# wustl-cig/FLAIR

Hardware: AMD Instinct MI355X
Metric: restored frames/sec at 256x256, 16-frame clip, 250-step DDIM (higher is better)
Workload: dtype bf16

## Files before the change

flair_amd/csrc/ew.hip:

```cpp
#include "common.h"

namespace {

template <typename E>
__global__ void nchw_to_nhwc_kernel(const float* src, int N, int C, long HW, E* dst, int ld, int coff) {
    const long total = (long)N * HW;
    for (long i = blockIdx.x * (long)blockDim.x + threadIdx.x; i < total; i += (long)gridDim.x * blockDim.x) {
        const long n = i / HW, p = i % HW;
        for (int c = 0; c < C; ++c) ET<E>::st(dst + i * ld + coff + c, src[(n * C + c) * HW + p]);
    }
}

template <typename E>
__global__ void nhwc_to_nchw_kernel(const E* src, int ld, int coff, int N, int C, long HW, float* dst) {
    const long total = (long)N * HW;
    for (long i = blockIdx.x * (long)blockDim.x + threadIdx.x; i < total; i += (long)gridDim.x * blockDim.x) {
        const long n = i / HW, p = i % HW;
        for (int c = 0; c < C; ++c) dst[(n * C + c) * HW + p] = ET<E>::ld(src + i * ld + coff + c);
    }
}

__global__ void timestep_embedding_kernel(const float* t, int N, int dim, float maxPeriod, int sinFirst,
                                          float* out) {
    const int half = dim / 2;
    const int i = blockIdx.x * blockDim.x + threadIdx.x;
    if (i >= N * half) return;
    const int n = i / half, k = i % half;
    const float freq = expf(-logf(maxPeriod) * (float)k / (float)half);
    const float arg = t[n] * freq;
    out[(long)n * dim + (sinFirst ? half : 0) + k] = cosf(arg);
    out[(long)n * dim + (sinFirst ? 0 : half) + k] = sinf(arg);
    if ((dim & 1) && k == 0) out[(long)n * dim + dim - 1] = 0.f;
}

template <int MMAX>
__global__ void linear_f32_kernel(const float* x, int M, int K, const float* w, const float* b, int N, int fpw,
                                  int actIn, int actOut, float* y, int yLd) {
    extern __shared__ float xs[];
    for (int i = threadIdx.x; i < M * K; i += blockDim.x) xs[i] = apply_act(x[i], actIn);
    __syncthreads();
    const int lane = threadIdx.x & 63;
    const int n0 = (blockIdx.x * (blockDim.x >> 6) + (threadIdx.x >> 6)) * fpw;
    for (int n = n0; n < n0 + fpw && n < N; ++n) {
        float acc[MMAX];
#pragma unroll
        for (int m = 0; m < MMAX; ++m) acc[m] = 0.f;
        const float* wr = w + (long)n * K;
        for (int k0 = lane; k0 < K; k0 += 64 * 8) {
            float wv[8];
#pragma unroll
            for (int j = 0; j < 8; ++j) wv[j] = k0 + 64 * j < K ? wr[k0 + 64 * j] : 0.f;
#pragma unroll
            for (int j = 0; j < 8; ++j) {
                const int k = k0 + 64 * j < K ? k0 + 64 * j : 0;
#pragma unroll
                for (int m = 0; m < MMAX; ++m)
                    if (m < M) acc[m] = fmaf(xs[m * K + k], wv[j], acc[m]);
            }
        }
#pragma unroll
        for (int m = 0; m < MMAX; ++m) {
            float v = acc[m];
#pragma unroll
            for (int off = 32; off > 0; off >>= 1) v += __shfl_xor(v, off);
            if (lane == 0 && m < M) y[(long)m * yLd + n] = apply_act(v + (b ? b[n] : 0.f), actOut);
        }
    }
}

__global__ void predict_xstart_kernel(const float* x, const float* modelOut, int N, int C, int Cm, long HW,
                                      float cRecip, float cRecipm1, int clip, float* x0) {
    const long total = (long)N * C * HW;
    for (long i = blockIdx.x * (long)blockDim.x + threadIdx.x; i < total; i += (long)gridDim.x * blockDim.x) {
        const long n = i / (C * HW), r = i % (C * HW);
        const float eps = modelOut[n * Cm * HW + r];
        float v = cRecip * x[i] - cRecipm1 * eps;
        if (clip) v = fminf(fmaxf(v, -1.f), 1.f);
        x0[i] = v;
    }
}

__global__ void sampler_update_kernel(const float* x, float* x0, const float* restored, const float* aux,
                                      const float* z, const float* prev, long frameElems, int T, int Tp,
                                      long total, float gamma, float wAux, float cRecip,
                                      float cRecipm1, float cPrev, float coNoise, float sq1mRho, float sqRho,
                                      int clip, int nonzero, float* xPrev) {
    for (long i = blockIdx.x * (long)blockDim.x + threadIdx.x; i < total; i += (long)gridDim.x * blockDim.x) {
        float v = x0[i];
        if (restored) {
            v = v - gamma * restored[i];
            if (clip) v = fminf(fmaxf(v, -1.f), 1.f);
        }
        if (aux) {
            float f = aux[i];
            if (clip) f = fminf(fmaxf(f, -1.f), 1.f);
            v = wAux * v + (1.f - wAux) * f;
        }
        if (prev) {
            const long n = i / frameElems, r = i % frameElems;
            const long b = n / T;
            const int t = (int)(n % T);
            if (t < Tp) v = prev[(b * Tp + t) * frameElems + r];
        }
        x0[i] = v;
        const float xi = x[i];
        const float eps = (cRecip * xi - v) / cRecipm1;
        float out = cPrev * v;
        if (nonzero) out += sq1mRho * coNoise * eps + sqRho * coNoise * z[i];
        xPrev[i] = out;
    }
}

__global__ void axpby_kernel(const float* x, const float* y, float a, float b, float lo, float hi, long n,
                             float* out) {
    for (long i = blockIdx.x * (long)blockDim.x + threadIdx.x; i < n; i += (long)gridDim.x * blockDim.x)
        out[i] = fminf(fmaxf(a * x[i] + (y ? b * y[i] : 0.f), lo), hi);
}

template <typename E>
__global__ void scale_pixels_kernel(E* x, int ld, int C, long P, const float* wmap) {
    constexpr int VEC = ET<E>::VEC;
    const int cv = C / VEC;
    const long total = P * cv;
    for (long i = blockIdx.x * (long)blockDim.x + threadIdx.x; i < total; i += (long)gridDim.x * blockDim.x) {
        const long p = i / cv;
        const int c0 = (int)(i % cv) * VEC;
        float v[VEC];
        Vec16<E>::load(x + p * ld + c0, v);
        const float s = wmap[p];
#pragma unroll
        for (int k = 0; k < VEC; ++k) v[k] *= s;
        Vec16<E>::store(x + p * ld + c0, v);
    }
}


__global__ void affine_channels_kernel(const float* x, int xLd, int C, long P, float a, float b, float lo,
                                       float hi, const float* sub, const float* mul, float* y, int yLd) {
    const long total = P * C;
    for (long i = blockIdx.x * (long)blockDim.x + threadIdx.x; i < total; i += (long)gridDim.x * blockDim.x) {
        const long p = i / C;
        const int c = (int)(i % C);
        float v = fminf(fmaxf(x[p * xLd + c] * a + b, lo), hi);
        y[p * yLd + c] = (v - (sub ? sub[c] : 0.f)) * (mul ? mul[c] : 1.f);
    }
}

template <typename E>
__global__ void add_frame_bias_kernel(E* x, int ld, int C, int F, long HW, const float* bias, int bLd) {
// ... 53 lines not shown
            Vec16<E>::load(x1 + p * ld1 + c0, b);
#pragma unroll
            for (int k = 0; k < VEC; ++k) a[k] += b[k];
        }
#pragma unroll
        for (int k = 0; k < VEC; ++k) a[k] = apply_act(a[k], act);
        Vec16<E>::store(y + p * yLd + c0, a);
    }
}

template <typename E>
__global__ void maxpool3s2_kernel(const E* x, int xLd, int F, int H, int W, int C, E* y, int yLd) {
    constexpr int VEC = ET<E>::VEC;
    const int cv = C / VEC, Ho = (H + 1) / 2, Wo = (W + 1) / 2;
    const long total = (long)F * Ho * Wo * cv;
    for (long i = blockIdx.x * (long)blockDim.x + threadIdx.x; i < total; i += (long)gridDim.x * blockDim.x) {
        const int c0 = (int)(i % cv) * VEC;
        long q = i / cv;
        const int wo = (int)(q % Wo);
        q /= Wo;
        const int ho = (int)(q % Ho), f = (int)(q / Ho);
        float m[VEC];
#pragma unroll
        for (int k = 0; k < VEC; ++k) m[k] = -INFINITY;
        for (int dh = -1; dh <= 1; ++dh) {
            const int h = 2 * ho + dh;
            if ((unsigned)h >= (unsigned)H) continue;
            for (int dw = -1; dw <= 1; ++dw) {
                const int w = 2 * wo + dw;
                if ((unsigned)w >= (unsigned)W) continue;
                float v[VEC];
                Vec16<E>::load(x + (((long)f * H + h) * W + w) * xLd + c0, v);
#pragma unroll
                for (int k = 0; k < VEC; ++k) m[k] = fmaxf(m[k], v[k]);
            }
        }
        Vec16<E>::store(y + (((long)f * Ho + ho) * Wo + wo) * yLd + c0, m);
    }
}

}

extern "C" int flair_nchw_f32_to_nhwc(const float* src, int N, int C, int H, int W, void* dst, int dtype,
                                      int dst_ld, int dst_coff, hipStream_t stream) {
    FLAIR_CHECK(src && dst && N > 0 && C > 0 && H > 0 && W > 0 && dst_coff >= 0 && dst_coff + C <= dst_ld,
                "flair_nchw_f32_to_nhwc: bad argument");
    const long HW = (long)H * W;
    return flair_by_dtype("flair_nchw_f32_to_nhwc", dtype, [&](auto e) -> int {
        using E = decltype(e);
        hipLaunchKernelGGL(nchw_to_nhwc_kernel<E>, dim3(grid_for(N * HW, 256, 2048)), dim3(256), 0, stream, src, N, C, HW,
                           (E*)dst, dst_ld, dst_coff);
        FLAIR_LAUNCH_CHECK();
        return FLAIR_OK;
    });
}

extern "C" int flair_nhwc_to_nchw_f32(const void* src, int dtype, int src_ld, int src_coff, int N, int C, int H,
                                      int W, float* dst, hipStream_t stream) {
    FLAIR_CHECK(src && dst && N > 0 && C > 0 && H > 0 && W > 0 && src_coff >= 0 && src_coff + C <= src_ld,
                "flair_nhwc_to_nchw_f32: bad argument");
    const long HW = (long)H * W;
    return flair_by_dtype("flair_nhwc_to_nchw_f32", dtype, [&](auto e) -> int {
        using E = decltype(e);
        hipLaunchKernelGGL(nhwc_to_nchw_kernel<E>, dim3(grid_for(N * HW, 256, 2048)), dim3(256), 0, stream,
                           (const E*)src, src_ld, src_coff, N, C, HW, dst);
        FLAIR_LAUNCH_CHECK();
        return FLAIR_OK;
    });
}

extern "C" int flair_timestep_embedding(const float* t, int N, int dim, float max_period, int sin_first,
                                        float* out, hipStream_t stream) {
    FLAIR_CHECK(t && out && N > 0 && dim >= 2, "flair_timestep_embedding: bad argument");
    const int n = N * (dim / 2);
    hipLaunchKernelGGL(timestep_embedding_kernel, dim3((n + 255) / 256), dim3(256), 0, stream, t, N, dim, max_period,
                       sin_first, out);
    FLAIR_LAUNCH_CHECK();
    return FLAIR_OK;
}

extern "C" int flair_linear_f32(const float* x, int M, int K, const float* w, const float* bias, int N, int act_in,
                                int act_out, float* y, int y_ld, hipStream_t stream) {
    FLAIR_CHECK(x && w && y && M > 0 && M <= 32 && K > 0 && N > 0 && y_ld >= N, "flair_linear_f32: bad argument (M<=32)");
    const size_t lds = (size_t)M * K * sizeof(float);
    FLAIR_CHECK(lds <= 64 * 1024, "flair_linear_f32: M*K too large for LDS staging");
    const int wavesPerBlock = 4;
    const int fpw = N >= 8192 ? 8 : 1;
    const int grid = (N + wavesPerBlock * fpw - 1) / (wavesPerBlock * fpw);
    if (M <= 8)
        hipLaunchKernelGGL(linear_f32_kernel<8>, dim3(grid), dim3(256), lds, stream, x, M, K, w, bias, N, fpw,
                           act_in, act_out, y, y_ld);
    else if (M <= 16)
        hipLaunchKernelGGL(linear_f32_kernel<16>, dim3(grid), dim3(256), lds, stream, x, M, K, w, bias, N, fpw,
                           act_in, act_out, y, y_ld);
    else
        hipLaunchKernelGGL(linear_f32_kernel<32>, dim3(grid), dim3(256), lds, stream, x, M, K, w, bias, N, fpw,
                           act_in, act_out, y, y_ld);
    FLAIR_LAUNCH_CHECK();
    return FLAIR_OK;
}

extern "C" int flair_predict_xstart(const float* x, const float* model_out, int N, int C, int Cm, int H, int W,
                                    float c_recip, float c_recipm1, int clip, float* x0, hipStream_t stream) {
    FLAIR_CHECK(x && model_out && x0 && N > 0 && C > 0 && Cm >= C, "flair_predict_xstart: bad argument");
    const long HW = (long)H * W;
    hipLaunchKernelGGL(predict_xstart_kernel, dim3(grid_for((long)N * C * HW, 256, 2048)), dim3(256), 0, stream, x, model_out, N,
                       C, Cm, HW, c_recip, c_recipm1, clip, x0);
    FLAIR_LAUNCH_CHECK();
    return FLAIR_OK;
}

extern "C" int flair_sampler_update(const flair_sampler_coefs* c, const float* x, float* x0, const float* restored,
                                    const float* aux, const float* z, const float* prev_recon, long n,
                                    float* x_prev, hipStream_t stream) {
    FLAIR_CHECK(c && x && x0 && x_prev && n > 0, "flair_sampler_update: null argument");
    FLAIR_CHECK(!c->nonzero || z, "flair_sampler_update: noise required when t != 0");
    FLAIR_CHECK(!prev_recon || (c->frame_elems > 0 && c->frames > 0 && c->prev_frames > 0 &&
                                c->prev_frames <= c->frames && n % (c->frame_elems * c->frames) == 0),
                "flair_sampler_update: prev_recon geometry");
    hipLaunchKernelGGL(sampler_update_kernel, dim3(grid_for(n, 256, 2048)), dim3(256), 0, stream, x, x0, restored, aux, z,
                       prev_recon, (long)c->frame_elems, c->frames, c->prev_frames, n,
                       c->gamma, c->w_aux, c->sqrt_recip_alphas_cumprod, c->sqrt_recipm1_alphas_cumprod,
                       c->sqrt_alphas_cumprod_prev, c->sqrt_one_minus_alphas_cumprod_prev, c->sqrt_one_minus_rho,
                       c->sqrt_rho, c->clip_denoised, c->nonzero, x_prev);
    FLAIR_LAUNCH_CHECK();
    return FLAIR_OK;
}

extern "C" int flair_axpby_f32(const float* x, const float* y, float a, float b, float lo, float hi, long n,
                               float* out, hipStream_t stream) {
    FLAIR_CHECK(x && out && n > 0, "flair_axpby_f32: bad argument");
    hipLaunchKernelGGL(axpby_kernel, dim3(grid_for(n, 256, 2048)), dim3(256), 0, stream, x, y, a, b, lo, hi, n, out);
    FLAIR_LAUNCH_CHECK();
    return FLAIR_OK;
}

extern "C" int flair_scale_pixels(void* x, int dtype, int ld, int C, long P, const float* wmap, hipStream_t stream) {
    FLAIR_CHECK(x && wmap && P > 0 && C > 0, "flair_scale_pixels: bad argument");
    return flair_by_dtype("flair_scale_pixels", dtype, [&](auto e) -> int {
        using E = decltype(e);
        constexpr int VEC = ET<E>::VEC;
        FLAIR_CHECK_VIEW("flair_scale_pixels", "x", x, ld, C, VEC);
        FLAIR_CHECK(C % VEC == 0, "flair_scale_pixels: C %% %d", VEC);
        hipLaunchKernelGGL(scale_pixels_kernel<E>, dim3(grid_for(P * (C / VEC), 256, 2048)), dim3(256), 0, stream, (E*)x, ld, C, P,
                           wmap);
        FLAIR_LAUNCH_CHECK();
        return FLAIR_OK;
    });
}

extern "C" int flair_affine_channels_f32(const float* x, int x_ld, int C, long P, float a, float b, float lo,
                                         float hi, const float* sub, const float* mul, float* y, int y_ld,
                                         hipStream_t stream) {
    FLAIR_CHECK(x && y && C > 0 && P > 0 && x_ld >= C && y_ld >= C, "flair_affine_channels_f32: bad argument");
    hipLaunchKernelGGL(affine_channels_kernel, dim3(grid_for(P * C, 256, 2048)), dim3(256), 0, stream, x, x_ld, C, P, a, b, lo,
                       hi, sub, mul, y, y_ld);
    FLAIR_LAUNCH_CHECK();
    return FLAIR_OK;
}

extern "C" int flair_add_frame_bias(void* x, int dtype, int ld, int C, int F, long HW, const float* bias,
                                    int bias_ld, hipStream_t stream) {
    FLAIR_CHECK(x && bias && C > 0 && F > 0 && HW > 0 && ld >= C && bias_ld >= C, "flair_add_frame_bias: bad argument");
    return flair_by_dtype("flair_add_frame_bias", dtype, [&](auto e) -> int {
        using E = decltype(e);
        hipLaunchKernelGGL(add_frame_bias_kernel<E>, dim3(grid_for(F * HW * C, 256, 2048)), dim3(256), 0, stream, (E*)x, ld, C, F,
                           HW, bias, bias_ld);
        FLAIR_LAUNCH_CHECK();
        return FLAIR_OK;
    });
}

extern "C" int flair_cast_channels(const float* src, int src_ld, int C, long P, void* dst, int dtype, int dst_ld,
                                   int dst_coff, hipStream_t stream) {
    FLAIR_CHECK(src && dst && C > 0 && P > 0 && src_ld >= C && dst_coff >= 0 && dst_coff + C <= dst_ld,
                "flair_cast_channels: bad argument");
    return flair_by_dtype("flair_cast_channels", dtype, [&](auto e) -> int {
        using E = decltype(e);
        hipLaunchKernelGGL(cast_channels_kernel<E>, dim3(grid_for(P * C, 256, 2048)), dim3(256), 0, stream, src, src_ld, C, P,
                           (E*)dst, dst_ld, dst_coff);
        FLAIR_LAUNCH_CHECK();
// ... 82 lines not shown
```

flair_amd/guided_diffusion/clip_model.py:

```python
import torch

from .packing import PackedModel


class ClipModel(PackedModel):

    _name = "flair_amd.ClipModel"

    def __init__(self, *args, **kwargs):
        super().__init__(*args, **kwargs)
        self._flow_cache = {}
        self._graphs = {}
        self.use_hip_graph = False
        self._flow_gen = 0
        self._trace = None

    def enable_hip_graph(self, flag=True):
        self.use_hip_graph = bool(flag)
        self._graphs = {}
        return self

    convert_to_fp16 = PackedModel.convert_to_bf16

    def invalidate_packed(self):
        super().invalidate_packed()
        self._graphs, self._flow_cache = {}, {}

    def reset_flow_cache(self):
        self._flow_cache = {}
        self._flow_gen += 1

    def _flows_cached(self, rnn_clip, spec):
        key = (rnn_clip.data_ptr(), rnn_clip._version, tuple(rnn_clip.shape), spec)
        hit = self._flow_cache.get(key)
        if hit is None:
            flows = self._compute_flows(rnn_clip, spec)
            flows["_prop"] = {}
            if len(self._flow_cache) >= 16:
                self._flow_cache.clear()
            hit = (flows, rnn_clip)
            self._flow_cache[key] = hit
        return hit[0]

    def _clip_flows(self, rnn_clip, x, enable_cross_frames):
        spec = self._flow_spec(x.shape[-2], x.shape[-1], enable_cross_frames)
        return self._flows_cached(rnn_clip, spec) if spec else {}

    def _run_clips(self, x, timesteps, low_res_input, rnn_input, num_frames, enable_cross_frames, vsrpp_weights):
        if not x.is_cuda:
            raise RuntimeError(f"{self._name} runs on the MI355X only (tensors must be on 'cuda'); "
                               "there is no CPU path")
        self._ensure_packed(x.device)
        T = int(num_frames)
        B = x.shape[0] // T
        if rnn_input is None:
            rnn_input = low_res_input
        graphed = self.use_hip_graph and self._trace is None
        outs = []
        for b in range(B):
            xb, tb = (v[b * T:(b + 1) * T].float().contiguous() for v in (x, timesteps))
            lr, rnn = (v[b].float().contiguous() for v in (low_res_input, rnn_input))
            vw = vsrpp_weights[b] if isinstance(vsrpp_weights, torch.Tensor) else vsrpp_weights
            if graphed:
                outs.append(self._forward_clip_graphed(xb, tb, lr, rnn, enable_cross_frames, vw, b))
            else:
                outs.append(self._forward_clip(xb, tb, lr, self._clip_flows(rnn, xb, enable_cross_frames),
                                               enable_cross_frames, vw))
        return outs[0] if B == 1 else torch.cat(outs, dim=0)

    def _forward_clip_graphed(self, x, t, low_res, rnn, enable_cross_frames, vsrpp_weights, clip):
        vw_t = vsrpp_weights if isinstance(vsrpp_weights, torch.Tensor) else None
        key = (tuple(x.shape), self.dtype, bool(enable_cross_frames),
               tuple(vw_t.shape) if vw_t is not None else vsrpp_weights, x.device, clip)
        src = (rnn.data_ptr(), rnn._version, low_res.data_ptr(), low_res._version, self._flow_gen,
               (vw_t.data_ptr(), vw_t._version) if vw_t is not None else None)
        ent = self._graphs.get(key)
        if ent is not None and ent["src"] != src:
            del self._graphs[key]
            ent = None
        if ent is None:
            st = dict(x=x.clone(), t=t.clone(), lr=low_res.clone(), rnn=rnn.clone(),
                      vw=vw_t.clone() if vw_t is not None else vsrpp_weights)
            flows = self._clip_flows(st["rnn"], x, enable_cross_frames)
            args = (st["x"], st["t"], st["lr"], flows, enable_cross_frames, st["vw"])
            cur = torch.cuda.current_stream()
            side = torch.cuda.Stream()
            side.wait_stream(cur)
            with torch.cuda.stream(side):
                self._forward_clip(*args)
            cur.wait_stream(side)
            torch.cuda.synchronize()
            graph = torch.cuda.CUDAGraph()
            with torch.cuda.graph(graph, capture_error_mode="thread_local"):
                out = self._forward_clip(*args)
            ent = dict(graph=graph, st=st, out=out, src=src, flows=flows)
            self._graphs[key] = ent
        ent["st"]["x"].copy_(x)
        ent["st"]["t"].copy_(t)
        ent["graph"].replay()
        return ent["out"]
```

flair_amd/guided_diffusion/sr3.py:

```python
import numpy as np
import torch
import torch.nn as nn

from .. import ops
from .clip_model import ClipModel
from .nn_new import linear, zero_module
from .packing import LinearStack, dev_f32, pack_w, packed_conv, pk_int, run_conv
from .unet_new import A, BasicVSRPP, Ctx, PlaceHolder, SPyNet, TemporalAttention, normalization

LazyReshaper2D = LazyReshaper3D = PlaceHolder


def aa_bilinear_table(n_in, n_out):
    scale = n_in / n_out
    support = scale if scale >= 1.0 else 1.0
    inv = 1.0 / scale if scale >= 1.0 else 1.0
    rows_i, rows_w = [], []
    for i in range(n_out):
        center = scale * (i + 0.5)
        lo = max(int(center - support + 0.5), 0)
        hi = min(int(center + support + 0.5), n_in)
        js = np.arange(lo, hi)
        w = np.clip(1.0 - np.abs((js - center + 0.5) * inv), 0.0, None).astype(np.float32)
        w = w / w.sum()
# ... 251 lines not shown
        self._shared_spynet = [shared]
        e = inner_channel
        self.noise_level_mlp = nn.Sequential(PositionalEncoding(inner_channel), nn.Linear(inner_channel, inner_channel * 4),
                                             Swish(), nn.Linear(inner_channel * 4, inner_channel))

        def blk(cin, cout, res):
            return ResnetBlocWithAttn(
                cin, cout, noise_level_emb_dim=e, norm_groups=norm_groups, dropout=dropout, conv_3d=cross_frame_module,
                temporal_attn=(res in attn_res and temporal_attn and cross_frame_module), num_frames=num_frames,
                head_dim=head_dim, vsrpp=(res in vsrpp_res and cross_frame_module),
                shared_spynet=shared if (res in vsrpp_res and cross_frame_module) else None)

        pre, res = inner_channel, image_size
        feats = [pre]
        downs = [LazyReshaper2D(nn.Conv2d(in_channel, inner_channel, kernel_size=3, padding=1))]
        n = len(channel_mults)
        for i in range(n):
            ch = inner_channel * channel_mults[i]
            for _ in range(res_blocks):
                downs.append(blk(pre, ch, res))
                feats.append(ch)
                pre = ch
            if i != n - 1:
                downs.append(LazyReshaper2D(Downsample(pre)))
                feats.append(pre)
                res //= 2
        self.downs = nn.ModuleList(downs)
        mk = dict(noise_level_emb_dim=e, norm_groups=norm_groups, dropout=dropout, conv_3d=cross_frame_module,
                  temporal_attn=temporal_attn and cross_frame_module, num_frames=num_frames, head_dim=head_dim)
        self.mid = nn.ModuleList([ResnetBlocWithAttn(pre, pre, **mk), ResnetBlocWithAttn(pre, pre, **mk)])
        ups, self._skip_split = [], {}
        for i in reversed(range(n)):
            ch = inner_channel * channel_mults[i]
            for _ in range(res_blocks + 1):
                skip = feats.pop()
                b = blk(pre + skip, ch, res)
                self._skip_split[id(b.res_block)] = [pre, skip]
                ups.append(b)
                pre = ch
            if i >= 1:
                ups.append(LazyReshaper2D(Upsample(pre)))
                res *= 2
        self.ups = nn.ModuleList(ups)
        self.final_conv = Block(pre, out_channel if out_channel is not None else in_channel, groups=norm_groups)

    def _pack_all(self, dt, device):
        stem = self.downs[0].wrapped_module
        stem._pk = packed_conv(stem, None, dt, device)
        plain, silu = LinearStack(), LinearStack()
        for m in self.modules():
            if isinstance(m, ResnetBlock):
                m.pack(dt, device, self._skip_split.get(id(m)), plain_off=plain.add(m.noise_func.noise_func[0]))
            elif isinstance(m, (ResBlock, TemporalWrapper2)):
                m.pack(dt, device, silu_off=silu.add(m.emb_layers[1]))
            elif isinstance(m, (TemporalAttention, BasicVSRPP, Downsample, Upsample)):
                m.pack(dt, device)
        if self._shared_spynet[0] is not None:
            self._shared_spynet[0].to(device)
            self._shared_spynet[0].pack(dt, device)
        mlp, fc = self.noise_level_mlp, self.final_conv.block
        self._pk = dict(
            plain=plain.cat(device), silu=silu.cat(device),
            mlp=[dev_f32(p, device) for p in (mlp[1].weight, mlp[1].bias, mlp[3].weight, mlp[3].bias)],
            fin_g=dev_f32(fc[0].wrapped_module.weight, device), fin_b=dev_f32(fc[0].wrapped_module.bias, device),
            fin=packed_conv(fc[3].wrapped_module, None, dt, device))
        self._flow_cache = {}

    def _flow_spec(self, H, W, enable_cross_frames):
        return tuple(self._flow_resolutions(H, W)) if enable_cross_frames else ()

    def _compute_flows(self, rnn_clip, resolutions):
        flows = {}
        for rh, r in resolutions:
            src = rnn_clip if tuple(rnn_clip.shape[-2:]) == (rh, r) else aa_resize(rnn_clip, (rh, r))
            raw = torch.zeros((src.shape[0], rh, r, 4), dtype=torch.float32, device=src.device)
            ops.nchw_to_clip(src.contiguous(), raw, 0)
            flows[r] = self._shared_spynet[0].pair_flows(raw)
        return flows

    def forward(self, x, timesteps, low_res_input=None, rnn_input=None, num_frames=None,
                enable_cross_frames=True, vsrpp_weights=None, **kwargs):
        return self._run_clips(x, timesteps, low_res_input, rnn_input, num_frames, enable_cross_frames, vsrpp_weights)

    def _forward_clip(self, x, level, low_res, flows, enable_cross_frames, vsrpp_weights):
        T, _, H, W = x.shape
        dev, dt = x.device, self.dtype
        ctx = Ctx(dt, dev, T)
        ctx.enable_cross_frames = enable_cross_frames
        ctx.vsrpp_weights = vsrpp_weights
        ctx.flows = flows
        pe = ops.timestep_embedding(level, self.inner_channel, sin_first=True)
        pk = self._pk
        e = ops.linear(pe, pk["mlp"][0], pk["mlp"][1], act_out=A.ACT_SILU)
        emb = ops.linear(e, pk["mlp"][2], pk["mlp"][3])
        ctx.plain_all = ops.linear(emb, pk["plain"][0], pk["plain"][1])
        ctx.silu_all = ops.linear(emb, pk["silu"][0], pk["silu"][1], act_in=A.ACT_SILU)
        cin = ops.pad_channels(self.in_channel, dt)
        h = torch.zeros((T, H, W, cin), dtype=dt, device=dev)
        ops.nchw_to_clip(low_res, h, 0)
        ops.nchw_to_clip(x, h, low_res.shape[1])
        feats = []
        for layer in self.downs:
            h = self._run_layer(ctx, layer, h)
            feats.append(h)
        for layer in self.mid:
            h = layer.run(ctx, h)
        for layer in self.ups:
            if isinstance(layer, ResnetBlocWithAttn):
                h = layer.run(ctx, h, feats.pop())
            else:
                h = self._run_layer(ctx, layer, h)
        fc = self.final_conv
        h = ops.group_norm(h, pk["fin_g"], pk["fin_b"], groups=fc.groups, eps=fc.block[0].wrapped_module.eps, act=A.ACT_SILU)
        y = run_conv(h, pk["fin"], fc.block[3].wrapped_module)
        return ops.clip_to_nchw(y, fc.block[3].wrapped_module.out_channels)

    def _flow_resolutions(self, H, W):
        hs, ws = ([r for r, _ in self._vsrpp_levels(n)] for n in (H, W))
        return sorted(set(zip(hs, ws)), key=lambda p: p[1])

    def _vsrpp_levels(self, size):
        out, res = [], size
        for layer in self.downs:
            if isinstance(layer, ResnetBlocWithAttn):
                if hasattr(layer, "vsrpp"):
                    out.append((res, layer.vsrpp.wrapped_module))
            elif isinstance(layer.wrapped_module, Downsample):
                res //= 2
        for layer in self.ups:
            if isinstance(layer, ResnetBlocWithAttn):
                if hasattr(layer, "vsrpp"):
                    out.append((res, layer.vsrpp.wrapped_module))
            elif isinstance(layer.wrapped_module, Upsample):
                res *= 2
        return out

    def _run_layer(self, ctx, layer, h):
        if isinstance(layer, ResnetBlocWithAttn):
            return layer.run(ctx, h)
        inner = layer.wrapped_module
        if isinstance(inner, nn.Conv2d):
            return run_conv(h, inner._pk, inner)
        if isinstance(inner, (Downsample, Upsample)):
            return inner.run(h)
        raise TypeError(f"flair_amd: no executor for {type(inner).__name__}")
```

flair_amd/guided_diffusion/unet_new.py:

```python
import math

import torch
import torch.nn as nn

from .. import ops
from .clip_model import ClipModel
from .nn_new import conv_nd, linear, normalization, zero_module
from .packing import LinearStack, dev_f32, pack_w, packed_conv, pk_int, run_conv

A = ops


class PlaceHolder(nn.Module):

    def __init__(self, module):
        super().__init__()
        self.wrapped_module = module


LazyReshaper2D = LazyReshaper3D = PlaceHolder


class TemporalWrapper(PlaceHolder):
    """unet_new.py:50-59 (skipped when ``enable_cross_frames`` is False)."""


class Ctx:

    def __init__(self, dtype, device, T):
        self.dtype, self.device, self.T = dtype, device, T
        self.emb = None
        self.film_all = None
        self.flows = {}
        self.vsrpp_weights = None
        self.enable_cross_frames = True


class ResBlock(nn.Module):

    def __init__(self, channels, emb_channels, dropout, out_channels=None, use_conv=False,
                 use_scale_shift_norm=False, dims=2, use_checkpoint=False, up=False, down=False):
        super().__init__()
        if not use_scale_shift_norm:
            raise NotImplementedError("flair_amd: only use_scale_shift_norm=True (the shipped "
                                      "FLAIR configuration) is implemented")
        if use_conv:
            raise NotImplementedError("flair_amd: 3x3 skip convolutions are not used by FLAIR")
        self.channels = channels
        self.out_channels = out_channels or channels
        self.dims, self.up, self.down = dims, up, down
        self.in_layers = nn.Sequential(
            PlaceHolder(normalization(channels)), nn.SiLU(),
            PlaceHolder(conv_nd(dims, channels, self.out_channels, 3, padding=1)))
        self.emb_layers = nn.Sequential(nn.SiLU(), linear(emb_channels, 2 * self.out_channels))
        self.out_layers = nn.Sequential(
            PlaceHolder(normalization(self.out_channels)), nn.SiLU(), nn.Dropout(p=dropout),
            zero_module(PlaceHolder(conv_nd(dims, self.out_channels, self.out_channels, 3, padding=1))))
        if self.out_channels == channels:
            self.skip_connection = nn.Identity()
        else:
            self.skip_connection = PlaceHolder(conv_nd(dims, channels, self.out_channels, 1))

    film_off = pk_int("film_off")

    def pack(self, dtype, device, split=None, film_off=0):
        c, co = self.channels, self.out_channels
        segs = [(s, s) for s in (split or [c])]
        self._pk = dict(
            film_off=film_off,
            w1=pack_w(self.in_layers[2].wrapped_module.weight, dtype, device, [(c, c)]),
            b1=dev_f32(self.in_layers[2].wrapped_module.bias, device),
            w2=pack_w(self.out_layers[3].wrapped_module.weight, dtype, device, [(co, co)]),
            b2=dev_f32(self.out_layers[3].wrapped_module.bias, device),
            g1=dev_f32(self.in_layers[0].wrapped_module.weight, device),
            be1=dev_f32(self.in_layers[0].wrapped_module.bias, device),
            g2=dev_f32(self.out_layers[0].wrapped_module.weight, device),
            be2=dev_f32(self.out_layers[0].wrapped_module.bias, device))
        if not isinstance(self.skip_connection, nn.Identity):
            self._pk["ws"] = pack_w(self.skip_connection.wrapped_module.weight, dtype, device, segs)
            self._pk["bs"] = dev_f32(self.skip_connection.wrapped_module.bias, device)

    def run(self, ctx, x, x1=None):
        pk = self._pk
        co = self.out_channels
        k = (1, 3, 3) if self.dims == 2 else (3, 3, 3)
        film = ctx.film_all[:, pk["film_off"]:pk["film_off"] + 2 * co]
        eps = self.in_layers[0].wrapped_module.eps
        if self.up or self.down:
            assert x1 is None
            h, x = ops.group_norm(x, pk["g1"], pk["be1"], eps=eps, act=A.ACT_SILU,
                                  resample=2 if self.up else 1, want_raw=True)
        else:
            h = ops.group_norm(x, pk["g1"], pk["be1"], x1=x1, eps=eps, act=A.ACT_SILU)
        h = ops.conv(h, pk["w1"], pk["b1"], co, k)
        h = ops.group_norm(h, pk["g2"], pk["be2"], eps=eps, act=A.ACT_SILU, film=film)
        if "ws" in pk:
            skip = ops.conv([x] if x1 is None else [x, x1], pk["ws"], pk["bs"], co, (1, 1, 1))
        else:
            assert x1 is None
            skip = x
        return ops.conv(h, pk["w2"], pk["b2"], co, k, res0=skip)


QKV_ATTN_WIDTHS = (32, 64, 128)


def qkv_head_width(channels, num_heads):
    d = channels // num_heads if num_heads > 0 and channels % num_heads == 0 else 0
    if d <= 0 or d % 8:
        raise NotImplementedError(f"flair_amd: attention head width {channels}/{num_heads} unsupported "
                                  f"({QKV_ATTN_WIDTHS} and multiples of 64 from 192 to 1024 at any size, other "
                                  "multiples of 8 while width + H*W <= 2048)")
    return d


def temporal_head_width(channels, num_heads):
    d = channels // num_heads if num_heads > 0 and channels % num_heads == 0 else 0
    if d < 8 or d > 256 or d % 8:
# ... 141 lines not shown
                    w1=pack_w(rb.conv1.weight, dtype, device, [(c, c)]), b1=dev_f32(rb.conv1.bias, device),
                    w2=pack_w(rb.conv2.weight, dtype, device, [(c, c)]), b2=dev_f32(rb.conv2.bias, device))




def run_trunk(pk, segs, c, *, extra_res=None, out=None, out_scale=1.0):
    k = (1, 3, 3)
    t1 = ops.conv(segs, pk["w0"], pk["b0"], c, k, act=A.ACT_LRELU01)
    if c == 64 and ops.chain_supported(t1, c):
        return ops.conv_chain(t1, pk["w1"], pk["b1"], A.ACT_RELU, pk["w2"], pk["b2"], A.ACT_NONE, c, c,
                              res0=t1, res1=extra_res, out=out, out_scale=out_scale)
    t2 = ops.conv(t1, pk["w1"], pk["b1"], c, k, act=A.ACT_RELU)
    return ops.conv(t2, pk["w2"], pk["b2"], c, k, res0=t1, res1=extra_res, out=out, out_scale=out_scale)


class SecondOrderDeformableAlignment(nn.Module):

    def __init__(self, in_channels, out_channels, kernel_size=3, padding=1, deform_groups=16,
                 max_residue_magnitude=10):
        super().__init__()
        assert kernel_size == 3 and padding == 1
        self.in_channels, self.out_channels = in_channels, out_channels
        self.deform_groups, self.max_residue_magnitude = deform_groups, max_residue_magnitude
        self.weight = nn.Parameter(torch.empty(out_channels, in_channels, 3, 3))
        self.bias = nn.Parameter(torch.zeros(out_channels))
        stdv = 1.0 / math.sqrt(in_channels * 9)
        with torch.no_grad():
            self.weight.uniform_(-stdv, stdv)
        c = out_channels
        self.conv_offset = nn.Sequential(
            nn.Conv2d(3 * c + 4, c, 3, 1, 1), nn.LeakyReLU(negative_slope=0.1),
            nn.Conv2d(c, c, 3, 1, 1), nn.LeakyReLU(negative_slope=0.1),
            nn.Conv2d(c, c, 3, 1, 1), nn.LeakyReLU(negative_slope=0.1),
            nn.Conv2d(c, 27 * deform_groups, 3, 1, 1))
        zero_module(self.conv_offset[-1])

    def pack(self, dtype, device):
        c = self.out_channels
        ka = ops.k_align(dtype)
        co = self.conv_offset
        perm = ops.dcn_raw_permutation(self.deform_groups)
        w6, b6 = co[6].weight.detach()[perm], co[6].bias.detach()[perm]
        return dict(
            w0=pack_w(co[0].weight, dtype, device, [(c, c), (c, c), (c, c), (4, ka)]), b0=dev_f32(co[0].bias, device),
            w2=pack_w(co[2].weight, dtype, device, [(c, c)]), b2=dev_f32(co[2].bias, device),
            w4=pack_w(co[4].weight, dtype, device, [(c, c)]), b4=dev_f32(co[4].bias, device),
            w6=pack_w(w6, dtype, device, [(c, c)]), b6=dev_f32(b6, device),
            wd=pack_w(self.weight, dtype, device, [(2 * c, 2 * c)]), bd=dev_f32(self.bias, device))


class BasicVSRPP(nn.Module):

    def __init__(self, mid_channels=64, max_residue_magnitude=10, use_checkpoint=False):
        super().__init__()
        self.mid_channels = mid_channels
        self.deform_align = nn.ModuleDict()
        self.backbone = nn.ModuleDict()
        for i, name in enumerate(["backward_1", "forward_1"]):
            self.deform_align[name] = SecondOrderDeformableAlignment(
                2 * mid_channels, mid_channels, 3, padding=1, deform_groups=16,
                max_residue_magnitude=max_residue_magnitude)
            self.backbone[name] = ResidualBlocksWithInputConv((2 + i) * mid_channels, mid_channels, 1)
        self.reconstruction = ResidualBlocksWithInputConv(3 * mid_channels, mid_channels, 1)
        self.conv_last = zero_module(nn.Conv2d(mid_channels, mid_channels, 1, 1))

    def pack(self, dtype, device):
        c = self.mid_channels
        self._pk = dict(
            align={n: m.pack(dtype, device) for n, m in self.deform_align.items()},
            trunk={"backward_1": self.backbone["backward_1"].pack(dtype, device, [c, c]),
                   "forward_1": self.backbone["forward_1"].pack(dtype, device, [c, c, c])},
            recon=self.reconstruction.pack(dtype, device, [c, c, c]),
            wl=pack_w(self.conv_last.weight, dtype, device, [(c, c)]), bl=dev_f32(self.conv_last.bias, device))

    def _propagate(self, ctx, hidden, flows, name, others, weight, wmaps, dest):
        pk_a, pk_t = self._pk["align"][name], self._pk["trunk"][name]
        T, H, W, c = hidden.shape
        order = list(range(T))
        flow_idx = list(range(-1, T - 1))
        if "backward" in name:
            order = order[::-1]
            flow_idx = order
        zero_c = torch.zeros((1, H, W, c), dtype=ctx.dtype, device=ctx.device)
        ka = ops.k_align(ctx.dtype)
        k3 = (1, 3, 3)
        G = self.deform_align[name].deform_groups
        mag = float(self.deform_align[name].max_residue_magnitude)
        store = ctx.flows.get("_prop") if isinstance(ctx.flows, dict) else None
        key = (name, H, W, ctx.dtype, ka)
        cached = store.get(key) if store is not None else None
        fill = [] if (cached is None and store is not None) else None
        prop, prev2 = zero_c, None
        for i, idx in enumerate(order):
            cur = hidden[idx:idx + 1]
            if i > 0:
                flow_n1 = flows[flow_idx[i]:flow_idx[i] + 1]
                cond_n1 = torch.empty_like(zero_c)
                second = i > 1
                feat_n2 = prev2 if second else zero_c
                cond_n2 = torch.empty_like(zero_c) if second else zero_c
                if cached is not None:
                    flow_n2, flowpad = cached[i - 1]
                    ops.vsrpp_warp2(prop, feat_n2 if second else None, flow_n1, flow_n2, cond_n1, cond_n2 if second else None)
                else:
                    flowpad = torch.zeros((1, H, W, ka), dtype=ctx.dtype, device=ctx.device)
                    flow_n2 = torch.empty_like(flow_n1) if second else None
                    ops.vsrpp_prep(prop, feat_n2 if second else None, flow_n1,
                                   flows[flow_idx[i - 1]:flow_idx[i - 1] + 1] if second else None,
                                   cond_n1, cond_n2 if second else None, flow_n2, flowpad)
                    if fill is not None:
                        fill.append((flow_n2, flowpad))
                o = ops.conv([cond_n1, cur, cond_n2, flowpad], pk_a["w0"], pk_a["b0"], c, k3, act=A.ACT_LRELU01)
                if c == 64 and ops.chain_supported(o, c):
                    o = ops.conv_chain(o, pk_a["w2"], pk_a["b2"], A.ACT_LRELU01, pk_a["w4"], pk_a["b4"],
                                       A.ACT_LRELU01, c, c)
                else:
                    o = ops.conv(o, pk_a["w2"], pk_a["b2"], c, k3, act=A.ACT_LRELU01)
                    o = ops.conv(o, pk_a["w4"], pk_a["b4"], c, k3, act=A.ACT_LRELU01)
                if c == 64 and ops.chain_supported(o, c) and W % 32 == 0:
                    raw = ops.conv_chain(o, None, None, A.ACT_NONE, pk_a["w6"], pk_a["b6"], A.ACT_DCN_OFFSETS, c, 27 * G,
                                         act_param=mag, act_period=3 * G)
                else:
                    raw = ops.conv(o, pk_a["w6"], pk_a["b6"], 27 * G, k3, act=A.ACT_DCN_OFFSETS, act_param=mag,
                                   act_period=3 * G)
                aligned = ops.dcn_align(prop, feat_n2, raw, flow_n1, flow_n2, pk_a["wd"], pk_a["bd"], c,
                                        groups=G, max_mag=mag, raw_activated=True)

            else:
                aligned = zero_c
            segs = [cur] + [o_[idx:idx + 1] for o_ in others] + [aligned]
            new = run_trunk(pk_t, segs, c, extra_res=aligned, out=dest[idx:idx + 1], out_scale=weight)
            if wmaps is not None:
                ops.scale_pixels(new, wmaps[idx])
            prev2, prop = (prop if i > 0 else None), new
        if fill is not None:
            store[key] = fill
        return dest

    def run(self, ctx, hidden):
        T, H, W, c = hidden.shape
        flows_forward, flows_backward = ctx.flows[W]
        weight, wmaps = 1.0, None
        vw = ctx.vsrpp_weights
        if isinstance(vw, (float, int)):
            weight = float(vw)
        elif vw is not None:
            wm = vw.reshape(T, vw.shape[-2], vw.shape[-1], 1).float().contiguous()
            if wm.shape[1] != H or wm.shape[2] != W:
                wm = ops.resize(wm, (H, W), ops.RESIZE_NEAREST)
            wmaps = [wm[i] for i in range(T)]
        bwd = torch.empty_like(hidden)
        fwd = torch.empty_like(hidden)
        self._propagate(ctx, hidden, flows_backward, "backward_1", [], weight, wmaps, bwd)
        ff = flows_forward if flows_forward is not None else flows_backward.flip(0)
        self._propagate(ctx, hidden, ff, "forward_1", [bwd], weight, wmaps, fwd)
        rec = run_trunk(self._pk["recon"], [hidden, bwd, fwd], c)
        return ops.conv(rec, self._pk["wl"], self._pk["bl"], c, (1, 1, 1), res0=hidden)


class _ConvModule(nn.Module):
    def __init__(self, cin, cout):
        super().__init__()
        self.conv = nn.Conv2d(cin, cout, kernel_size=7, stride=1, padding=3)


class SPyNetBasicModule(nn.Module):
# ... 150 lines not shown
                ch = cout
                chans.append(ch)
            if level != len(channel_mult) - 1:
                self.input_blocks.append(TimestepEmbedSequential(res(ch, ch, down=True)))
                chans.append(ch)
                ds *= 2
        ident = nn.Identity
        self.middle_block = TimestepEmbedSequential(
            res(ch, ch),
            TemporalWrapper(res(ch, ch, 3)) if temporal_block else ident(),
            AttentionbottleBlock(ch, use_checkpoint=use_checkpoint, num_heads=num_heads,
                                 num_head_channels=num_head_channels,
                                 use_new_attention_order=use_new_attention_order),
            TemporalWrapper(TemporalAttention(ch, 5, num_heads, num_head_channels, use_checkpoint))
            if temporal_block else ident(),
            res(ch, ch),
            TemporalWrapper(res(ch, ch, 3)) if temporal_block else ident())
        self._skip_split = []
        self.output_blocks = nn.ModuleList([])
        for level, mult in list(enumerate(channel_mult))[::-1]:
            for i in range(num_res_blocks + 1):
                ich = chans.pop()
                cout = int(model_channels * mult)
                layers = level_layers(ch + ich, cout, ds, num_heads_upsample)
                self._skip_split.append((ch, ich))
                ch = cout
                if level and i == num_res_blocks:
                    layers.append(res(ch, ch, up=True))
                    ds //= 2
                self.output_blocks.append(TimestepEmbedSequential(*layers))
        self.out = nn.Sequential(LazyReshaper3D(normalization(ch)), nn.SiLU(),
                                 zero_module(LazyReshaper2D(conv_nd(dims, input_ch, out_channels, 3, padding=1))))

    def _pack_all(self, dt, device):
        stem = self.input_blocks[0][0].wrapped_module
        stem._pk = packed_conv(stem, None, dt, device)
        first_out = {id(st[0]): split for st, split in zip(self.output_blocks, self._skip_split)}
        film = LinearStack()
        for m in self.modules():
            has_film = isinstance(m, ResBlock) or (isinstance(m, AttentionBlock) and m.bottleneck)
            off = film.add(m.emb_layers[1]) if has_film else 0
            if isinstance(m, ResBlock):
                m.pack(dt, device, list(first_out[id(m)]) if id(m) in first_out else None, film_off=off)
            elif isinstance(m, AttentionBlock):
                m.pack(dt, device, film_off=off)
            elif isinstance(m, (TemporalAttention, BasicVSRPP, SPyNet)):
                m.pack(dt, device)
        emb_w, emb_b = film.cat(device)
        self._pk = dict(
            emb_w=emb_w, emb_b=emb_b,
            te=[dev_f32(p, device) for p in (self.time_embed[0].weight, self.time_embed[0].bias,
                                            self.time_embed[2].weight, self.time_embed[2].bias)],
            head_g=dev_f32(self.out[0].wrapped_module.weight, device), head_b=dev_f32(self.out[0].wrapped_module.bias, device),
            head=packed_conv(self.out[2].wrapped_module, None, dt, device))
        self._flow_cache = {}

    def compute_flow(self, lqs):
        T, _, h, w = lqs.shape
        raw = torch.zeros((T, h, w, 4), dtype=torch.float32, device=lqs.device)
        ops.nchw_to_clip(lqs.contiguous(), raw, 0)
        return self.spynet.pair_flows(raw)

    def _flow_spec(self, H, W, enable_cross_frames):
        return (H, W)

    def _compute_flows(self, rnn_clip, hw):
        T, _, h, w = rnn_clip.shape
        H, W = hw
        raw = torch.zeros((T, h, w, 4), dtype=torch.float32, device=rnn_clip.device)
        ops.nchw_to_clip(rnn_clip.contiguous(), raw, 0)
        flows = {}
        for s in self.rnn_resolutions:
            if H % s or W % s:
                raise ValueError(f"{self._name}: a {H}x{W} clip has no level at down-sampling {s}")
            rh, rw = H // s, W // s
            src = raw if (h, w) == (rh, rw) else ops.resize(raw, (rh, rw), ops.RESIZE_BICUBIC, channels=3)
            flows[rw] = self.spynet.pair_flows(src)
        return flows

    def forward(self, x, timesteps, low_res_input=None, num_frames=None, rnn_input=None,
                enable_cross_frames=True, vsrpp_weights=None, **kwargs):
        return self._run_clips(x, timesteps, low_res_input, rnn_input, num_frames, enable_cross_frames, vsrpp_weights)

    def _forward_clip(self, x, t, low_res, flows, enable_cross_frames, vsrpp_weights):
        T, _, H, W = x.shape
        dev, dt = x.device, self.dtype
        ctx = Ctx(dt, dev, T)
        ctx.enable_cross_frames = enable_cross_frames
        ctx.vsrpp_weights = vsrpp_weights
        ctx.flows = flows
        temb = ops.timestep_embedding(t, self.model_channels)
        pk = self._pk
        e = ops.linear(temb, pk["te"][0], pk["te"][1], act_out=A.ACT_SILU)
        ctx.emb = ops.linear(e, pk["te"][2], pk["te"][3])
        ctx.film_all = ops.linear(ctx.emb, pk["emb_w"], pk["emb_b"], act_in=A.ACT_SILU)
        cin = ops.pad_channels(self.in_channels, dt)
        h = torch.zeros((T, H, W, cin), dtype=dt, device=dev)
        ops.nchw_to_clip(x, h, 0)
        ops.nchw_to_clip(low_res.contiguous(), h, x.shape[1])
        hs = []
        trace = self._trace
        for i, blk in enumerate(self.input_blocks):
            h = blk.run(ctx, h)
            hs.append(h)
            if trace is not None:
                trace.append((f"input_blocks.{i}", h))
        h = self.middle_block.run(ctx, h)
        if trace is not None:
            trace.append(("middle_block", h))
        for i, blk in enumerate(self.output_blocks):
            h = blk.run(ctx, h, hs.pop())
            if trace is not None:
                trace.append((f"output_blocks.{i}", h))
        h = ops.group_norm(h, pk["head_g"], pk["head_b"], eps=self.out[0].wrapped_module.eps, act=A.ACT_SILU)
        y = run_conv(h, pk["head"], self.out[2].wrapped_module)
        return ops.clip_to_nchw(y, self.out_channels)
```

Baseline: 0.8599.

## Pipeline weight prefetch in small-M linear kernel and cache stem input and zero buffers

The small-M linear kernel now triple-buffers its weight-row loads in registers and holds the activation slice in registers. It reduces all rows with a butterfly bpermute, launches at most 2048 wave tasks, and splits M into chunks of 16 rows. The model also caches the low-res stem tensor (low-res channels written once per clip, keyed by pointer and version) and reuses zero tensors in the propagation loop, removing per-step allocations and copies. The stem cache writes x into the cached buffer in place, so reuse relies on the x channels being fully overwritten each call. The version key guards against stale low-res data.

```diff
diff --git a/flair_amd/csrc/ew.hip b/flair_amd/csrc/ew.hip
--- a/flair_amd/csrc/ew.hip
+++ b/flair_amd/csrc/ew.hip
@@ -1,3 +1,5 @@
+#include <type_traits>
+
 #include "common.h"
 
 namespace {
@@ -34,37 +36,94 @@
 }
 
 template <int MMAX>
-__global__ void linear_f32_kernel(const float* x, int M, int K, const float* w, const float* b, int N, int fpw,
-                                  int actIn, int actOut, float* y, int yLd) {
+__global__ __launch_bounds__(256, 2) void linear_f32_kernel(const float* x, int M, int K, const float* w, const float* b,
+                                                            int N, int fpw, int actIn, int actOut, float* y, int yLd) {
     extern __shared__ float xs[];
-    for (int i = threadIdx.x; i < M * K; i += blockDim.x) xs[i] = apply_act(x[i], actIn);
+    const int lane = threadIdx.x & 63;
+    const int n0 = (blockIdx.x * 4 + __builtin_amdgcn_readfirstlane(threadIdx.x >> 6)) * fpw;
+    const int n1 = n0 + fpw < N ? n0 + fpw : N;
+    const int nkb = (K + 511) >> 9;
+
+    int fn = n0, fkb = 0;
+    auto fetch = [&](float (&wv)[9]) __attribute__((always_inline)) {
+        const int f = fn < N ? fn : N - 1;
+        const float* wr = w + (long)f * K;
+        const int k0 = fkb * 512 + lane;
+#pragma unroll
+        for (int j = 0; j < 8; ++j) wv[j] = wr[k0 + 64 * j < K ? k0 + 64 * j : K - 1];
+        wv[8] = (b ? b : w)[f];
+        if (++fkb == nkb) {
+            fkb = 0;
+            ++fn;
+        }
+    };
+    float wa[9] = {}, wb[9] = {}, wc[9] = {};
+    fetch(wa);
+    fetch(wb);
+
+    for (int i0 = threadIdx.x; i0 < M * K; i0 += 256 * 16) {
+        float v[16];
+#pragma unroll
+        for (int u = 0; u < 16; ++u) v[u] = x[i0 + 256 * u < M * K ? i0 + 256 * u : M * K - 1];
+#pragma unroll
+        for (int u = 0; u < 16; ++u)
+            if (i0 + 256 * u < M * K) xs[i0 + 256 * u] = apply_act(v[u], actIn);
+    }
     __syncthreads();
-    const int lane = threadIdx.x & 63;
-    const int n0 = (blockIdx.x * (blockDim.x >> 6) + (threadIdx.x >> 6)) * fpw;
-    for (int n = n0; n < n0 + fpw && n < N; ++n) {
-        float acc[MMAX];
+
+    float xr[MMAX][8];
+    auto take_x = [&](int kb) __attribute__((always_inline)) {
+#pragma unroll
+        for (int j = 0; j < 8; ++j) {
+            const int kk = kb * 512 + lane + 64 * j;
+            const int k = kk < K ? kk : 0;
+#pragma unroll
+            for (int m = 0; m < MMAX; ++m) xr[m][j] = xs[(m < M ? m : M - 1) * K + k];
+        }
+    };
+    if (nkb == 1) take_x(0);
+
+    float acc[MMAX];
+#pragma unroll
+    for (int m = 0; m < MMAX; ++m) acc[m] = 0.f;
+    int n = n0, kb = 0;
+    auto step = [&](const float (&wv)[9], float (&refill)[9]) __attribute__((always_inline)) {
+        fetch(refill);
+        if (nkb > 1) take_x(kb);
+#pragma unroll
+        for (int j = 0; j < 8; ++j) {
+            const float wj = kb * 512 + lane + 64 * j < K ? wv[j] : 0.f;
+#pragma unroll
+            for (int m = 0; m < MMAX; ++m) acc[m] = fmaf(xr[m][j], wj, acc[m]);
+        }
+        if (++kb < nkb) return;
+        auto from = [&](float v, int off) { return __int_as_float(__builtin_amdgcn_ds_bpermute((lane ^ off) << 2, __float_as_int(v))); };
+        int row = 0;
+#pragma unroll
+        for (int s = 0; s < 6; ++s) {
+            const int off = 32 >> s, half = MMAX >> (s + 1);
+            const bool hi = lane & off;
+#pragma unroll
+            for (int i = 0; i < MMAX / 2; ++i) {
+                if (i >= half) continue;
+                const float lower = acc[i], upper = acc[i + half];
+                acc[i] = (hi ? upper : lower) + from(hi ? lower : upper, off);
+            }
+            if (half > 0 && hi) row += half;
+            if (half == 0) acc[0] += from(acc[0], off);
+        }
+        if ((lane & (64 / MMAX - 1)) == 0 && row < M) y[(long)row * yLd + n] = apply_act(acc[0] + (b ? wv[8] : 0.f), actOut);
 #pragma unroll
         for (int m = 0; m < MMAX; ++m) acc[m] = 0.f;
-        const float* wr = w + (long)n * K;
-        for (int k0 = lane; k0 < K; k0 += 64 * 8) {
-            float wv[8];
-#pragma unroll
-            for (int j = 0; j < 8; ++j) wv[j] = k0 + 64 * j < K ? wr[k0 + 64 * j] : 0.f;
-#pragma unroll
-            for (int j = 0; j < 8; ++j) {
-                const int k = k0 + 64 * j < K ? k0 + 64 * j : 0;
-#pragma unroll
-                for (int m = 0; m < MMAX; ++m)
-                    if (m < M) acc[m] = fmaf(xs[m * K + k], wv[j], acc[m]);
-            }
-        }
-#pragma unroll
-        for (int m = 0; m < MMAX; ++m) {
-            float v = acc[m];
-#pragma unroll
-            for (int off = 32; off > 0; off >>= 1) v += __shfl_xor(v, off);
-            if (lane == 0 && m < M) y[(long)m * yLd + n] = apply_act(v + (b ? b[n] : 0.f), actOut);
-        }
+        kb = 0;
+        ++n;
+    };
+    while (n < n1) {
+        step(wa, wc);
+        if (n >= n1) break;
+        step(wb, wa);
+        if (n >= n1) break;
+        step(wc, wb);
     }
 }
 
@@ -284,21 +343,29 @@
 extern "C" int flair_linear_f32(const float* x, int M, int K, const float* w, const float* bias, int N, int act_in,
                                 int act_out, float* y, int y_ld, hipStream_t stream) {
     FLAIR_CHECK(x && w && y && M > 0 && M <= 32 && K > 0 && N > 0 && y_ld >= N, "flair_linear_f32: bad argument (M<=32)");
-    const size_t lds = (size_t)M * K * sizeof(float);
-    FLAIR_CHECK(lds <= 64 * 1024, "flair_linear_f32: M*K too large for LDS staging");
-    const int wavesPerBlock = 4;
-    const int fpw = N >= 8192 ? 8 : 1;
-    const int grid = (N + wavesPerBlock * fpw - 1) / (wavesPerBlock * fpw);
-    if (M <= 8)
-        hipLaunchKernelGGL(linear_f32_kernel<8>, dim3(grid), dim3(256), lds, stream, x, M, K, w, bias, N, fpw,
-                           act_in, act_out, y, y_ld);
-    else if (M <= 16)
-        hipLaunchKernelGGL(linear_f32_kernel<16>, dim3(grid), dim3(256), lds, stream, x, M, K, w, bias, N, fpw,
-                           act_in, act_out, y, y_ld);
-    else
-        hipLaunchKernelGGL(linear_f32_kernel<32>, dim3(grid), dim3(256), lds, stream, x, M, K, w, bias, N, fpw,
-                           act_in, act_out, y, y_ld);
-    FLAIR_LAUNCH_CHECK();
+    const size_t lds = (size_t)(M < 16 ? M : 16) * K * sizeof(float);
+    FLAIR_CHECK(lds <= 160 * 1024, "flair_linear_f32: min(M, 16) * K = %zu floats too large for LDS staging (40960)", lds / 4);
+    const int fpw = (N + 2047) / 2048;
+    const int grid = (N + 4 * fpw - 1) / (4 * fpw);
+    for (int m0 = 0; m0 < M; m0 += 16) {
+        const int rows = M - m0 < 16 ? M - m0 : 16;
+        const float* xm = x + (size_t)m0 * K;
+        float* ym = y + (size_t)m0 * y_ld;
+        const size_t ldsRows = (size_t)rows * K * sizeof(float);
+        auto launch = [&](auto mmax) -> int {
+            constexpr int MMAX = decltype(mmax)::value;
+            static LdsAttrOnce attr;
+            FLAIR_CHECK(ldsRows <= 64 * 1024 ||
+                            flair_max_lds_once(attr, reinterpret_cast<const void*>(&linear_f32_kernel<MMAX>)) == hipSuccess,
+                        "flair_linear_f32: hipFuncSetAttribute failed");
+            hipLaunchKernelGGL(linear_f32_kernel<MMAX>, dim3(grid), dim3(256), ldsRows, stream, xm, rows, K, w, bias, N, fpw,
+                               act_in, act_out, ym, y_ld);
+            FLAIR_LAUNCH_CHECK();
+            return FLAIR_OK;
+        };
+        const int rc = rows <= 8 ? launch(std::integral_constant<int, 8>{}) : launch(std::integral_constant<int, 16>{});
+        if (rc != FLAIR_OK) return rc;
+    }
     return FLAIR_OK;
 }
 
diff --git a/flair_amd/guided_diffusion/clip_model.py b/flair_amd/guided_diffusion/clip_model.py
--- a/flair_amd/guided_diffusion/clip_model.py
+++ b/flair_amd/guided_diffusion/clip_model.py
@@ -10,6 +10,8 @@
     def __init__(self, *args, **kwargs):
         super().__init__(*args, **kwargs)
         self._flow_cache = {}
+        self._stem_cache = {}
+        self._consts = {}
         self._graphs = {}
         self.use_hip_graph = False
         self._flow_gen = 0
@@ -25,9 +27,11 @@
     def invalidate_packed(self):
         super().invalidate_packed()
         self._graphs, self._flow_cache = {}, {}
+        self._stem_cache, self._consts = {}, {}
 
     def reset_flow_cache(self):
         self._flow_cache = {}
+        self._stem_cache = {}
         self._flow_gen += 1
 
     def _flows_cached(self, rnn_clip, spec):
@@ -45,6 +49,16 @@
     def _clip_flows(self, rnn_clip, x, enable_cross_frames):
         spec = self._flow_spec(x.shape[-2], x.shape[-1], enable_cross_frames)
         return self._flows_cached(rnn_clip, spec) if spec else {}
+
+    def _stem_cached(self, x, low_res):
+        key = (low_res.data_ptr(), low_res._version, tuple(low_res.shape), tuple(x.shape), self.dtype, self._flow_gen)
+        hit = self._stem_cache.get(key)
+        if hit is None:
+            if len(self._stem_cache) >= 8:
+                self._stem_cache.clear()
+            hit = (self._stem_input(x, low_res), low_res)
+            self._stem_cache[key] = hit
+        return hit[0]
 
     def _run_clips(self, x, timesteps, low_res_input, rnn_input, num_frames, enable_cross_frames, vsrpp_weights):
         if not x.is_cuda:
@@ -64,8 +78,8 @@
             if graphed:
                 outs.append(self._forward_clip_graphed(xb, tb, lr, rnn, enable_cross_frames, vw, b))
             else:
-                outs.append(self._forward_clip(xb, tb, lr, self._clip_flows(rnn, xb, enable_cross_frames),
-                                               enable_cross_frames, vw))
+                outs.append(self._forward_clip(xb, tb, self._stem_cached(xb, lr),
+                                               self._clip_flows(rnn, xb, enable_cross_frames), enable_cross_frames, vw))
         return outs[0] if B == 1 else torch.cat(outs, dim=0)
 
     def _forward_clip_graphed(self, x, t, low_res, rnn, enable_cross_frames, vsrpp_weights, clip):
@@ -82,7 +96,8 @@
             st = dict(x=x.clone(), t=t.clone(), lr=low_res.clone(), rnn=rnn.clone(),
                       vw=vw_t.clone() if vw_t is not None else vsrpp_weights)
             flows = self._clip_flows(st["rnn"], x, enable_cross_frames)
-            args = (st["x"], st["t"], st["lr"], flows, enable_cross_frames, st["vw"])
+            st["stem"] = self._stem_input(st["x"], st["lr"])
+            args = (st["x"], st["t"], st["stem"], flows, enable_cross_frames, st["vw"])
             cur = torch.cuda.current_stream()
             side = torch.cuda.Stream()
             side.wait_stream(cur)
diff --git a/flair_amd/guided_diffusion/sr3.py b/flair_amd/guided_diffusion/sr3.py
--- a/flair_amd/guided_diffusion/sr3.py
+++ b/flair_amd/guided_diffusion/sr3.py
@@ -357,10 +357,16 @@
                 enable_cross_frames=True, vsrpp_weights=None, **kwargs):
         return self._run_clips(x, timesteps, low_res_input, rnn_input, num_frames, enable_cross_frames, vsrpp_weights)
 
-    def _forward_clip(self, x, level, low_res, flows, enable_cross_frames, vsrpp_weights):
+    def _stem_input(self, x, low_res):
         T, _, H, W = x.shape
+        h = torch.zeros((T, H, W, ops.pad_channels(self.in_channel, self.dtype)), dtype=self.dtype, device=x.device)
+        return ops.nchw_to_clip(low_res, h, 0)
+
+    def _forward_clip(self, x, level, stem, flows, enable_cross_frames, vsrpp_weights):
+        T = x.shape[0]
         dev, dt = x.device, self.dtype
         ctx = Ctx(dt, dev, T)
+        ctx.consts = self._consts
         ctx.enable_cross_frames = enable_cross_frames
         ctx.vsrpp_weights = vsrpp_weights
         ctx.flows = flows
@@ -370,10 +376,7 @@
         emb = ops.linear(e, pk["mlp"][2], pk["mlp"][3])
         ctx.plain_all = ops.linear(emb, pk["plain"][0], pk["plain"][1])
         ctx.silu_all = ops.linear(emb, pk["silu"][0], pk["silu"][1], act_in=A.ACT_SILU)
-        cin = ops.pad_channels(self.in_channel, dt)
-        h = torch.zeros((T, H, W, cin), dtype=dt, device=dev)
-        ops.nchw_to_clip(low_res, h, 0)
-        ops.nchw_to_clip(x, h, low_res.shape[1])
+        h = ops.nchw_to_clip(x, stem, self.in_channel - x.shape[1])
         feats = []
         for layer in self.downs:
             h = self._run_layer(ctx, layer, h)
diff --git a/flair_amd/guided_diffusion/unet_new.py b/flair_amd/guided_diffusion/unet_new.py
--- a/flair_amd/guided_diffusion/unet_new.py
+++ b/flair_amd/guided_diffusion/unet_new.py
@@ -34,6 +34,14 @@
         self.flows = {}
         self.vsrpp_weights = None
         self.enable_cross_frames = True
+        self.consts = {}
+
+    def zeros(self, *shape):
+        key = (shape, self.dtype, self.device)
+        z = self.consts.get(key)
+        if z is None:
+            z = self.consts[key] = torch.zeros(shape, dtype=self.dtype, device=self.device)
+        return z
 
 
 class ResBlock(nn.Module):
@@ -341,7 +349,7 @@
         if "backward" in name:
             order = order[::-1]
             flow_idx = order
-        zero_c = torch.zeros((1, H, W, c), dtype=ctx.dtype, device=ctx.device)
+        zero_c = ctx.zeros(1, H, W, c)
         ka = ops.k_align(ctx.dtype)
         k3 = (1, 3, 3)
         G = self.deform_align[name].deform_groups
@@ -658,10 +666,16 @@
                 enable_cross_frames=True, vsrpp_weights=None, **kwargs):
         return self._run_clips(x, timesteps, low_res_input, rnn_input, num_frames, enable_cross_frames, vsrpp_weights)
 
-    def _forward_clip(self, x, t, low_res, flows, enable_cross_frames, vsrpp_weights):
+    def _stem_input(self, x, low_res):
+        T, _, H, W = x.shape
+        h = torch.zeros((T, H, W, ops.pad_channels(self.in_channels, self.dtype)), dtype=self.dtype, device=x.device)
+        return ops.nchw_to_clip(low_res.contiguous(), h, x.shape[1])
+
+    def _forward_clip(self, x, t, stem, flows, enable_cross_frames, vsrpp_weights):
         T, _, H, W = x.shape
         dev, dt = x.device, self.dtype
         ctx = Ctx(dt, dev, T)
+        ctx.consts = self._consts
         ctx.enable_cross_frames = enable_cross_frames
         ctx.vsrpp_weights = vsrpp_weights
         ctx.flows = flows
@@ -670,10 +684,7 @@
         e = ops.linear(temb, pk["te"][0], pk["te"][1], act_out=A.ACT_SILU)
         ctx.emb = ops.linear(e, pk["te"][2], pk["te"][3])
         ctx.film_all = ops.linear(ctx.emb, pk["emb_w"], pk["emb_b"], act_in=A.ACT_SILU)
-        cin = ops.pad_channels(self.in_channels, dt)
-        h = torch.zeros((T, H, W, cin), dtype=dt, device=dev)
-        ops.nchw_to_clip(x, h, 0)
-        ops.nchw_to_clip(low_res.contiguous(), h, x.shape[1])
+        h = ops.nchw_to_clip(x, stem, 0)
         hs = []
         trace = self._trace
         for i, blk in enumerate(self.input_blocks):
```

After: 0.8658, median of 6. About the same (+0.7%).
